# Kudo510/ImageSequenceRegistrationfor6DPoseEstimationLabeling

Measured on AMD Instinct MI355X. Metric: registered images/sec (T-LESS obj 1-like, synthetic) + final Chamfer error, higher is better.
Workload: dtype bf16

## Files before the change

### imagesequenceregistrationfor6dposeestimationlabeling_amd/_capi.py

```python
from __future__ import annotations

import ctypes as C
from pathlib import Path

import torch

import os

_PKG = Path(__file__).resolve().parent
LIB_PATH = Path(os.environ["ISR_HIP_LIB"]) if os.environ.get("ISR_HIP_LIB") else _PKG / "libisr_hip.so"

ISR_OK = 0
ABI_VERSION = 6
DTYPE_BF16 = 0
DTYPE_F32 = 1
DTYPE_BF16_LOG2 = 2
DTYPE_BF16_LOG2_SCREENED = 3
RANSAC_STAGED = 0
RANSAC_SEQUENTIAL = 1
INLIERS_REFIT = 0
INLIERS_RANSAC = 1
FINAL_REFIT = 0
FINAL_EPNP = 1
TUNE = {"nn_path": 0, "nn_filter": 1, "icp_warm": 2, "nn_plan_rq": 3, "nn_plan_blocks": 4,
        "nn_tile_st": 5, "nn_tile_sq": 6, "nn_tile_tb": 7, "ep_wsum_valu": 8, "k1_f32_chain": 9, "k1_split": 10}


class IsrError(RuntimeError):
    pass


_lib = None

_vp = C.c_void_p
_i = C.c_int
_sz = C.c_size_t
_d = C.c_double
_f = C.c_float
_u64 = C.c_uint64
_i64 = C.c_int64

SIGNATURES = {
    "isr_abi_version": (_i, []),
    "isr_last_error": (C.c_char_p, []),
    "isr_device_count": (_i, []),
    "isr_tuning_set": (_i, [_i, _i]),
    "isr_tuning_get": (_i, [_i]),
    "isr_corr_argmax_workspace_bytes": (_sz, [_i, _i, _i, _i]),
    "isr_corr_argmax": (_i, [_vp, _vp, _i, _i, _i, _i, _i, _i, _vp, _vp, _vp, _vp, _sz, _vp]),
    "isr_corr_argmax_digits": (_i, [_vp, _vp, _i, _i, _i, _i, _i, _i, _vp, _vp, _vp, _i, _vp, _vp, _vp, _sz, _vp]),
    "isr_corr_argmax_phase": (_i, [_vp, _vp, _i, _i, _i, _i, _i, _i, _vp, _vp, _vp, _i, _vp, _vp, _i, _vp, _sz, _vp]),
    "isr_corr_argmax_recheck_count": (_i, [_vp, _sz, _i, _i, _i, _vp, _vp]),
    "isr_corr_argmax_recheck_count_f32": (_i, [_vp, _sz, _i, _i, _i, _vp, _vp]),
    "isr_corr_argmax_screen_redone": (_i, [_vp, _sz, _i, _i, _i, _vp, _vp]),
    "isr_corr_quantize_fp6": (_i, [_vp, _i, _i, _vp, _vp, _vp, _vp]),
    "isr_corr_argmax_clock_mhz": (_i, [_vp, _sz, _i, _i, _i, _vp, _vp]),
    "isr_adds_bounds": (_i, [_vp, _i, _vp, _vp, _i, _vp, _vp, _d, _i, _i, _i, _vp, _vp, _vp, _vp]),
    "isr_corr_topk_workspace_bytes": (_sz, [_i, _i]),
    "isr_corr_topk": (_i, [_vp, _vp, _i, _i, _i, _i, _i, _i, _vp, _vp, _vp, _vp, _sz, _vp]),
    "isr_corr_logsoftmax_workspace_bytes": (_sz, [_i, _i, _i, _i]),
    "isr_corr_logsoftmax": (_i, [_vp, _vp, _i, _i, _i, _i, _i, _i, _vp, _i64, _vp, _sz, _vp]),
    "isr_ep_corr_matrices": (_i, [_vp, _vp, _i, _i, _i, _vp, _vp, _vp, _sz, _vp]),
    "isr_mask_bbox": (_i, [_vp, _i, _i, _i, _i, _vp, _vp]),
    "isr_crop_normalize": (_i, [_vp, _vp, _i, _i, _i, _i, _vp, _i, _i, _vp, _vp, _vp, _vp, _vp]),
    "isr_select_top_batch_workspace_bytes": (_sz, [_i, _i]),
    "isr_select_top_batch": (_i, [_vp, _i, _i, _vp, _d, _i, _vp, _vp, _vp, _vp, _sz, _vp]),
# ... 115 lines not shown
```

### imagesequenceregistrationfor6dposeestimationlabeling_amd/csrc/capi_common.hip

```cpp
#include "isr_common.hpp"

#include <atomic>
#include <cstdlib>
#include <cstring>

namespace isr {

char* last_error_buf() {
  static thread_local char buf[512] = {0};
  return buf;
}

void set_error(const char* fmt, ...) {
  va_list ap;
  va_start(ap, fmt);
  vsnprintf(last_error_buf(), 512, fmt, ap);
  va_end(ap);
}

namespace {

struct Tuning {
  std::atomic<int> v[ISR_TUNE_COUNT];
  Tuning() {
    const int defaults[ISR_TUNE_COUNT] = {-1, -1, 1, 0, 0, 0, 0, 0, 0, 0, 0};
    for (int i = 0; i < ISR_TUNE_COUNT; ++i) v[i].store(defaults[i], std::memory_order_relaxed);
    if (const char* e = getenv("ISR_NN_GRID")) { if (e[0] >= '0' && e[0] <= '2') v[ISR_TUNE_NN_PATH] = e[0] - '0'; }
    if (const char* e = getenv("ISR_NN_FILTER")) { if (e[0] == '0' || e[0] == '1') v[ISR_TUNE_NN_FILTER] = e[0] - '0'; }
    if (const char* e = getenv("ISR_ICP_WARM")) { if (e[0] == '0') v[ISR_TUNE_ICP_WARM] = 0; }
    if (const char* e = getenv("ISR_NN_PLAN")) {
      int rq = 0; long want = 0;
      if (sscanf(e, "%d,%ld", &rq, &want) >= 1) {
        if (rq == 1 || rq == 4) v[ISR_TUNE_NN_PLAN_RQ] = rq;
        if (want > 0) v[ISR_TUNE_NN_PLAN_BLOCKS] = (int)want;
      }
    }
    if (const char* e = getenv("ISR_NN_TILE")) {
      double st = 0, sq = 0; int tb = 0;
      (void)sscanf(e, "%lf,%lf,%d", &st, &sq, &tb);
      if (st > 0) v[ISR_TUNE_NN_TILE_ST] = (int)(st * 1000.0 + 0.5);
// ... 97 lines not shown
```

### imagesequenceregistrationfor6dposeestimationlabeling_amd/csrc/corr_argmax.hip

```cpp
#include "isr_common.hpp"

#include <type_traits>

namespace {

using bf16x8 = __attribute__((ext_vector_type(8))) short;
using f16x8 = __attribute__((ext_vector_type(8))) _Float16;
using f32x16 = __attribute__((ext_vector_type(16))) float;

constexpr int kThreads = 256;
constexpr int kWaves = kThreads / 64;
constexpr int kQB = 2;
constexpr int kTK = 128;
constexpr int kChunkStages = 32;
constexpr int kChunk = kTK * kChunkStages;
constexpr float kLog2e = 1.4426950408889634f;
constexpr float kNoM2 = -1.0e30f;
constexpr int kKnBlocks = 64;
constexpr int kRSplitMax = 4;

struct CorrWs {
  float* pm;
  float* pm2;
  int32_t* pbi;
// ... 533 lines not shown
  constexpr int W = 16 * SP;
  const long i = (long)blockIdx.x * 256 + threadIdx.x;
  if (i >= (long)R * W) return;
  const long row = i / W;
  const int d = (int)(i % W);
  const float x = d < D ? X[row * ld + d] * prescale : 0.f;
  if (fabsf(x) > 65000.f) *ovf = 1;
  const _Float16 x1 = (_Float16)x;
  const float r = x - (float)x1;
  const _Float16 x2s = (_Float16)(r * 2048.f);
  const _Float16 x1s = (_Float16)((float)x1 * 4.8828125e-4f);
  uint16_t* o = out + row * (3 * W) + d;
  o[0] = __builtin_bit_cast(uint16_t, x1); o[W] = __builtin_bit_cast(uint16_t, x2s); o[2 * W] = __builtin_bit_cast(uint16_t, x1s);
}

template <bool F16 = false>
__global__ __launch_bounds__(256) void corr_keynorm_kernel(const uint16_t* __restrict__ K, int N, int D,
                                                           int ldk, float inflate, CorrWs ws) {
  __shared__ float red[4];
  if (ws.digits)
    for (int i = blockIdx.x * 256 + threadIdx.x; i < ws.ndigits; i += kKnBlocks * 256) ws.digits[i] = 0;
  if (gated_off(ws)) return;
  float mx = 0.f;
  for (int i = blockIdx.x * 256 + threadIdx.x; i < ws.nhand; i += kKnBlocks * 256) ws.hand[i] = 0;
  for (int n = blockIdx.x * 256 + threadIdx.x; n < N; n += kKnBlocks * 256) {
    const uint16_t* row = K + (size_t)n * ldk;
    float s = 0.f;
    for (int d = 0; d < D; d += 8) {
      const uint4 v = *reinterpret_cast<const uint4*>(row + d);
      const uint32_t w[4] = {v.x, v.y, v.z, v.w};
#pragma unroll
      for (int j = 0; j < 4; ++j) {
        const float lo = elem_f32<F16>((uint16_t)(w[j] & 0xFFFFu)), hi = elem_f32<F16>((uint16_t)(w[j] >> 16));
        s = __builtin_fmaf(lo, lo, s);
        s = __builtin_fmaf(hi, hi, s);
      }
    }
    mx = fmaxf(mx, s);
  }
#pragma unroll
  for (int o = 32; o >= 1; o >>= 1) mx = fmaxf(mx, __shfl_xor(mx, o, 64));
  if ((threadIdx.x & 63) == 0) red[threadIdx.x >> 6] = mx;
  __syncthreads();
  if (threadIdx.x == 0) {
    ws.kn2[blockIdx.x] = fmaxf(fmaxf(red[0], red[1]), fmaxf(red[2], red[3])) * inflate;
    if (blockIdx.x == 0) {
      ws.rcount[0] = 0; ws.rcount[1] = 0; ws.rcount[2] = 0; ws.rcount[3] = 0;
      if (ws.kmax) { ws.kmax[0] = 0u; ws.kmax[1] = 0u; ws.redone[0] = 0ull; ws.redone[1] = 0ull; }
    }
  }
}

__device__ __forceinline__ void digit_count(const CorrWs& ws, int q, float lp) {
  const int img = q / ws.rows_per_image, r = q - img * ws.rows_per_image;
  const bool valid = !ws.n_rows || r < ws.n_rows[img];
  const int key = valid ? img * isr::kDigitBins + (int)(isr::ordered_bits(lp) >> isr::kDigitShift) : -1;
  const int lane = (int)__builtin_amdgcn_mbcnt_hi(~0u, __builtin_amdgcn_mbcnt_lo(~0u, 0u));
  unsigned long long todo = __builtin_amdgcn_ballot_w64(valid);
  while (todo != 0ull) {
    const int leader = (int)__builtin_ctzll(todo);
    const int k = __builtin_amdgcn_readlane(key, leader);
    const unsigned long long same = __builtin_amdgcn_ballot_w64(key == k);
    if (lane == leader) atomicAdd(&ws.digits[k], (int)__builtin_popcountll(same));
    todo &= ~same;
  }
// ... 509 lines not shown
  uint16_t *q2, *k2;
  int32_t* gate;
  CorrWs ws;
  if (route.kind == 1) carve_split(w, P, N, &q2, &k2, &ws);
  else carve_planes(w, P, N, route.sp, route.kind == 3, &q2, &k2, &gate, &ws, nullptr);
  hipStream_t stream = isr::as_stream(stream_);
  int32_t gated = 0;
  if (route.kind == 3) ISR_CHECK_HIP(hipMemcpyAsync(&gated, gate, sizeof(int32_t), hipMemcpyDeviceToHost, stream));
  ISR_CHECK_HIP(hipMemcpyAsync(count_host, ws.rcount, sizeof(int32_t), hipMemcpyDeviceToHost, stream));
  ISR_CHECK_HIP(hipStreamSynchronize(stream));
  if (gated) *count_host = -1;
  return ISR_OK;
}

namespace {

int launch_bf16(const uint16_t* q, const uint16_t* k, int P, int N, int D, int ldq, int ldk, bool log2, const CorrPlan& p,
                const CorrWs& ws, int32_t* idx, float* logp, float* lse, F32Rows f32, float kn_inflate, hipStream_t stream,
                int sp = 0, bool f16 = false, bool screened = false, int phase = 3) {
  const bool ph1 = (phase & 1) != 0, ph2 = (phase & 2) != 0;
  const float eabs = (sp && f16) ? split_eabs(sp) : 0.f;
  const bool lse_only = idx == nullptr;
  const dim3 grid(p.qblocks, p.nsplit);
  const int fin_blocks = (P + 255) / 256;
  const int fin_bf16 = (p.nsplit == 1 && fin_blocks > kFallbackGrid) ? kFallbackGrid : fin_blocks;
  ISR_REQUIRE(sp != 0 || D == 16 || D == 32 || D == 64 || D == 128,
              "isr_corr_argmax(bf16): D=%d must be 16, 32, 64 or 128 (zero-pad the columns)", D);
  ISR_REQUIRE(ldq % 8 == 0 && ldk % 8 == 0 && ((uintptr_t)q % 16 == 0) && ((uintptr_t)k % 16 == 0),
              "isr_corr_argmax(bf16): rows must be 16-byte aligned (ldq=%d ldk=%d)", ldq, ldk);
  ISR_REQUIRE((long long)p.range_chunks * kChunk * ldk * 2 < (1ll << 31),
              "isr_corr_argmax(bf16): a key range of %d rows x ldk=%d exceeds the 2 GiB buffer window",
              p.range_chunks * kChunk, ldk);
  const int cgrid = (int)(((long)p.qblocks * p.nchunks < kFallbackGrid) ? (long)p.qblocks * p.nchunks : kFallbackGrid);
  const dim3 rgrid(16 * kRSplitGrid);
  const double scale = log2 ? 0.6931471805599453094 : 1.0;
  if (ph1) {
    if (f16) corr_keynorm_kernel<true><<<kKnBlocks, 256, 0, stream>>>(k, N, 16 * sp, ldk, kn_inflate, ws);
    else corr_keynorm_kernel<false><<<kKnBlocks, 256, 0, stream>>>(k, N, sp ? 16 * sp : D, ldk, kn_inflate, ws);
  }
#define ISR_LAUNCH_BF16(DKv)                                                                                  \
  do {                                                                                                        \
    if (log2) {                                                                                               \
      if (ph1) {                                                                                              \
      if (lse_only && DKv <= 2)    \
        corr_bf16_direct_kernel<DKv, kQB, false, DKv, 0, false, (DKv <= 2)><<<grid, kThreads, 0, stream>>>(q, k, P, N, ldq, ldk, \
                                                                              p.range_chunks, ws, idx, logp, lse); \
      else                                                                                                    \
      corr_bf16_direct_kernel<DKv, kQB, false><<<grid, kThreads, 0, stream>>>(q, k, P, N, ldq, ldk,          \
                                                                              p.range_chunks, ws, idx, logp, lse); \
      }                                                                                                       \
      if (ph2) {                                                                                              \
      corr_bf16_kernel<DKv, true><<<cgrid, kThreads, 0, stream>>>(q, k, P, N, ldq, ldk, p.range_chunks, p.qblocks,      \
                                                                  p.nchunks, ws);  \
// ... 212 lines not shown
                       false, dg.phase);
  }
  CorrPlan p = make_plan(P, N, slots_for(dtype, D), kWaves * kQB * 32);
  const bool screened = screened_route(dtype, N, D);
  if (screened) {
    p.nsplit = 1;
    p.range_chunks = p.nchunks;
  }
  isr::Workspace w(ws_, ws_bytes);
  CorrWs ws;
  carve(w, P, N, dtype, &ws);
  dg.apply(&ws);
  if (dtype != ISR_DTYPE_F32) {
    return launch_bf16(static_cast<const uint16_t*>(Q), static_cast<const uint16_t*>(K), P, N, D, ldq, ldk,
                       dtype != ISR_DTYPE_BF16, p, ws, idx, logp, lse, F32Rows{nullptr, nullptr, 0, 0, 0}, 1.f, stream, 0, false, screened,
                       dg.phase);
  }
  if (dg.hist && (dg.phase & 1))
    ISR_CHECK_HIP(hipMemsetAsync(dg.hist, 0, sizeof(int32_t) * (size_t)dg.images * isr::kDigitBins, stream));
  return launch_f32_chain(static_cast<const float*>(Q), static_cast<const float*>(K), P, N, D, ldq, ldk, p, ws, idx, logp, lse, stream,
                          dg.phase);
}

}

extern "C" int isr_corr_argmax(const void* Q, const void* K, int P, int N, int D, int ldq, int ldk,
                               int dtype, int32_t* idx, float* logp, float* lse, void* ws_,
                               size_t ws_bytes, isr_stream_t stream_) {
  return corr_argmax_impl(Q, K, P, N, D, ldq, ldk, dtype, idx, logp, lse, ws_, ws_bytes, stream_, DigitArgs{});
}

// ... 34 lines not shown
```

### imagesequenceregistrationfor6dposeestimationlabeling_amd/ops.py

```python
from __future__ import annotations

import ctypes
from dataclasses import dataclass

import numpy as np

import torch

from . import _capi
from ._capi import check, current_stream, lib, ptr, require_cuda

_workspaces: dict[tuple, torch.Tensor] = {}

_timers: dict[str, list] | None = None


def enable_timing(on: bool = True) -> None:
    global _timers
    _timers = {} if on else None


def drain_timing() -> dict[str, tuple[int, float, float]]:
    out = {}
    if _timers is None:
# ... 211 lines not shown
def _pad_cols(t: torch.Tensor, D: int) -> torch.Tensor:
    if t.shape[1] == D:
        return t.contiguous()
    out = torch.zeros((t.shape[0], D), dtype=t.dtype, device=t.device)
    out[:, : t.shape[1]] = t
    return out


LOG2E = 1.4426950408889634


def prescale_queries_log2(queries: torch.Tensor) -> torch.Tensor:
    return (queries.to(torch.float32) * LOG2E).to(torch.bfloat16)


@dataclass
class CorrCall:
    q: torch.Tensor
    k: torch.Tensor
    P: int
    N: int
    Dp: int
    dtype: int
    idx: torch.Tensor
    logp: torch.Tensor
    lse: torch.Tensor | None
    rows_per_image: int
    n_rows: torch.Tensor | None
    hist: torch.Tensor | None
    ws: torch.Tensor
    dev: torch.device

    def outputs(self):
        out = (self.idx, self.logp) if self.lse is None else (self.idx, self.logp, self.lse)
        return out if self.hist is None else out + (self.hist,)


def _corr_prepare(queries, keys, want_lse, log2_prescaled, screened, rows_per_image, n_rows, ws_tag) -> CorrCall:
    dev = require_cuda(queries, keys, n_rows)
    if queries.ndim != 2 or keys.ndim != 2 or queries.shape[1] != keys.shape[1]:
        raise ValueError(f"queries {tuple(queries.shape)} / keys {tuple(keys.shape)} must be (P,D),(N,D)")
    P, D = queries.shape
    N = keys.shape[0]
    if P == 0 or N == 0:
        raise ValueError("empty queries or keys")
    if screened and not log2_prescaled:
        raise ValueError("screened needs log2-prescaled bf16 queries")
    if queries.dtype == torch.bfloat16 and keys.dtype == torch.bfloat16:
        dtype = (_capi.DTYPE_BF16_LOG2_SCREENED if screened else _capi.DTYPE_BF16_LOG2) if log2_prescaled else _capi.DTYPE_BF16
        Dp = next((d for d in (16, 32, 64, 128) if d >= D), None)
        if Dp is None:
            raise ValueError(f"bf16 path supports D <= 128, got {D}")
    else:
        if log2_prescaled:
            raise ValueError("log2_prescaled needs bf16 queries and keys")
        dtype = _capi.DTYPE_F32
        queries, keys = queries.to(torch.float32), keys.to(torch.float32)
        Dp = D
        if D > 128:
            raise ValueError(f"f32 path supports D <= 128, got {D}")
    q, k = _pad_cols(queries, Dp), _pad_cols(keys, Dp)
    idx = torch.empty(P, dtype=torch.int32, device=dev)
    logp = torch.empty(P, dtype=torch.float32, device=dev)
    lse = torch.empty(P, dtype=torch.float32, device=dev) if want_lse else None
    ws = workspace(dev, lib().isr_corr_argmax_workspace_bytes(P, N, Dp, dtype), ws_tag)
    hist = None
    if rows_per_image is not None:
        if rows_per_image <= 0 or P % rows_per_image:
            raise ValueError(f"corr_argmax: P={P} is not a whole number of images of {rows_per_image} rows")
        if n_rows is not None and (n_rows.dtype != torch.int32 or n_rows.numel() != P // rows_per_image):
            raise ValueError("corr_argmax: n_rows must be (images,) int32")
        hist = torch.empty((P // rows_per_image, 2048), dtype=torch.int32, device=dev)
    return CorrCall(q, k, P, N, Dp, dtype, idx, logp, lse, int(rows_per_image or 1), n_rows, hist, ws, dev)


def _corr_launch(c: CorrCall, phase: int, what: str, work: float) -> None:
    L = lib()
    with torch.cuda.device(c.dev), _timed(what, work):
        if phase == 3 and c.hist is None:
            rc = L.isr_corr_argmax(ptr(c.q), ptr(c.k), c.P, c.N, c.Dp, c.Dp, c.Dp, c.dtype, ptr(c.idx), ptr(c.logp), ptr(c.lse),
                                   ptr(c.ws), c.ws.numel(), current_stream(c.dev))
        elif phase == 3:
            rc = L.isr_corr_argmax_digits(ptr(c.q), ptr(c.k), c.P, c.N, c.Dp, c.Dp, c.Dp, c.dtype, ptr(c.idx), ptr(c.logp), ptr(c.lse),
                                          c.rows_per_image, ptr(c.n_rows), ptr(c.hist), ptr(c.ws), c.ws.numel(), current_stream(c.dev))
        else:
            rc = L.isr_corr_argmax_phase(ptr(c.q), ptr(c.k), c.P, c.N, c.Dp, c.Dp, c.Dp, c.dtype, ptr(c.idx), ptr(c.logp), ptr(c.lse),
                                         c.rows_per_image, ptr(c.n_rows), ptr(c.hist), phase, ptr(c.ws), c.ws.numel(),
                                         current_stream(c.dev))
    check(rc, "isr_corr_argmax")
    global _last_corr
    _last_corr = (c.ws, c.P, c.N, c.dtype, c.dev)


def corr_argmax(queries: torch.Tensor, keys: torch.Tensor, want_lse: bool = False,
                log2_prescaled: bool = False, screened: bool = False, rows_per_image: int | None = None,
                n_rows: torch.Tensor | None = None):
    c = _corr_prepare(queries, keys, want_lse, log2_prescaled, screened, rows_per_image, n_rows, "corr")
    _corr_launch(c, 3, "corr_argmax", 2.0 * c.P * c.N * c.Dp)
    return c.outputs()


def corr_argmax_open(queries: torch.Tensor, keys: torch.Tensor, want_lse: bool = False, log2_prescaled: bool = False,
                     screened: bool = False, rows_per_image: int | None = None, n_rows: torch.Tensor | None = None,
                     ws_tag: str = "corr") -> CorrCall:
    c = _corr_prepare(queries, keys, want_lse, log2_prescaled, screened, rows_per_image, n_rows, ws_tag)
    _corr_launch(c, 1, "corr_argmax", 2.0 * c.P * c.N * c.Dp)
    return c


def corr_argmax_close(call: CorrCall):
    _corr_launch(call, 2, "corr_close", 0.0)
    return call.outputs()


def corr_lse(queries: torch.Tensor, keys: torch.Tensor, log2_prescaled: bool = False, screened: bool = False) -> torch.Tensor:
    dev = require_cuda(queries, keys)
    if queries.ndim != 2 or keys.ndim != 2 or queries.shape[1] != keys.shape[1]:
        raise ValueError(f"queries {tuple(queries.shape)} / keys {tuple(keys.shape)} must be (P,D),(N,D)")
    P, D = queries.shape
    N = keys.shape[0]
    if P == 0 or N == 0:
        raise ValueError("empty queries or keys")
    if queries.dtype == torch.bfloat16 and keys.dtype == torch.bfloat16:
        dtype = (_capi.DTYPE_BF16_LOG2_SCREENED if screened else _capi.DTYPE_BF16_LOG2) if log2_prescaled else _capi.DTYPE_BF16
        Dp = next((d for d in (16, 32, 64, 128) if d >= D), None)
        if Dp is None:
            raise ValueError(f"bf16 path supports D <= 128, got {D}")
    else:
        if log2_prescaled:
            raise ValueError("log2_prescaled needs bf16 queries and keys")
        dtype = _capi.DTYPE_F32
        queries, keys = queries.to(torch.float32), keys.to(torch.float32)
        Dp = D
        if D > 128:
            raise ValueError(f"f32 path supports D <= 128, got {D}")
    q, k = _pad_cols(queries, Dp), _pad_cols(keys, Dp)
    lse = torch.empty(P, dtype=torch.float32, device=dev)
    L = lib()
    ws = workspace(dev, L.isr_corr_argmax_workspace_bytes(P, N, Dp, dtype), "corr")
    with torch.cuda.device(dev), _timed("corr_lse", 2.0 * P * N * Dp):
        rc = L.isr_corr_argmax(ptr(q), ptr(k), P, N, Dp, Dp, Dp, dtype, None, None, ptr(lse), ptr(ws), ws.numel(),
                               current_stream(dev))
    check(rc, "isr_corr_argmax (lse only)")
    return lse


def corr_topk(queries: torch.Tensor, keys: torch.Tensor, k: int):
    dev = require_cuda(queries, keys)
    if queries.ndim != 2 or keys.ndim != 2 or queries.shape[1] != keys.shape[1]:
        raise ValueError(f"queries {tuple(queries.shape)} / keys {tuple(keys.shape)} must be (P,D),(N,D)")
    if not 1 <= int(k) <= 8:
# ... 554 lines not shown
```

### imagesequenceregistrationfor6dposeestimationlabeling_amd/sequence.py

```python
from __future__ import annotations

from dataclasses import dataclass

import numpy as np
import torch

from . import ops, pose_est_surf, pose_refine, registration, shard


@dataclass
class SequenceModel:
    keys: torch.Tensor
    pts: torch.Tensor
    log2_queries: bool = False
    screened: bool = False


EPILOGUE_DIGITS = False


@dataclass
class ImageResult:
    pose: torch.Tensor
    status: torch.Tensor
    n_inl: torch.Tensor
    inl_idx: torch.Tensor
    keep: torch.Tensor
    M: torch.Tensor
    idx: torch.Tensor
    logp: torch.Tensor
    n_eval: torch.Tensor | None = None


def register_image(model: SequenceModel, queries: torch.Tensor, pix_xy: torch.Tensor, cam,
                   itr: int = 500, reperr: float = 2.0, seed: int = 0, refine_iters: int = 10,
                   timing: list | None = None, confidence: float = 0.99, loop: str = "staged",
                   inliers: str = "refit", final: str = "refit") -> ImageResult:
    ops._loop_args(loop, inliers, None, final)
    if timing is not None:
        e0, e1 = torch.cuda.Event(enable_timing=True), torch.cuda.Event(enable_timing=True)
        e0.record()
    idx, logp = ops.corr_argmax(queries, model.keys, log2_prescaled=model.log2_queries, screened=model.screened and model.log2_queries)
    if timing is not None:
        e1.record()
        timing.append((e0, e1))
    keep, M, _ = ops.select_top(logp)
    p3d, p2d = ops.gather_corr(idx, keep, M, model.pts, pix_xy)
    r = ops.pnp_ransac(p3d, p2d, cam, H=itr, reperr=reperr, seed=seed, refine_iters=refine_iters, M_dev=M,
                       confidence=confidence, loop=loop, inliers=inliers, final=final)
    return ImageResult(r.pose, r.status, r.n_inl, r.inl_idx, keep, M, idx, logp, r.n_eval)


def register_crop(model: SequenceModel, feat: torch.Tensor, mask: torch.Tensor, cam, c0: int = 0,
                  n_feat: int | None = None, down_sample: int = 3, itr: int = 500, reperr: float = 2.0,
                  seed: int = 0, refine_iters: int = 10, confidence: float = 0.99, loop: str = "staged",
                  inliers: str = "refit", final: str = "refit") -> tuple[ImageResult, torch.Tensor]:
    ops._loop_args(loop, inliers, None, final)
    D = model.keys.shape[1] if n_feat is None else n_feat
    if model.keys.dtype == torch.bfloat16:
        dtype = "bf16_log2" if model.log2_queries else "bf16"
    else:
        dtype = "f32"
    Q, pix, n_dev = ops.prep_queries(feat, mask, c0=c0, D=D, step=down_sample, dtype=dtype)
    keys = model.keys if model.keys.shape[1] == Q.shape[1] else ops._pad_cols(model.keys, Q.shape[1])
    idx, logp = ops.corr_argmax(Q, keys, log2_prescaled=model.log2_queries, screened=model.screened and model.log2_queries)
    keep, M, _ = ops.select_top(logp, n_dev=n_dev)
    p3d, p2d = ops.gather_corr(idx, keep, M, model.pts, pix)
    r = ops.pnp_ransac(p3d, p2d, cam, H=itr, reperr=reperr, seed=seed, refine_iters=refine_iters, M_dev=M,
                       confidence=confidence, loop=loop, inliers=inliers, final=final)
    return ImageResult(r.pose, r.status, r.n_inl, r.inl_idx, keep, M, idx, logp, r.n_eval), n_dev


def register_frame(model: SequenceModel, rgb, mask, camparams, encoder, n_feat: int = 12, down_sample: int = 3,
                   itr: int = 500, reperr: float = 2.0, seed: int = 0, refine_iters: int = 10, confidence: float = 0.99,
                   useMask: bool = True, loop: str = "staged", inliers: str = "refit", final: str = "refit"):
    from . import registration
    ops._loop_args(loop, inliers, None, final)
    inputIM, cropMask, cam, _ = registration.crop_inputs(rgb, mask, camparams, useMask=useMask, down_sample=down_sample)
    with torch.no_grad():
        imfeatsfull = torch.movedim(encoder(inputIM), 1, 3)
# ... 14 lines not shown
    D = model.keys.shape[1] if n_feat is None else n_feat
    if model.keys.dtype == torch.bfloat16:
        dtype = "bf16_log2" if model.log2_queries else "bf16"
    else:
        dtype = "f32"
    cams = np.asarray(cams, np.float64)
    cams = np.broadcast_to(cams, (n, 3, 3)) if cams.ndim == 2 else cams
    seeds = list(range(n)) if seeds is None else list(seeds)
    cur = torch.cuda.current_stream(dev)
    serial = n_streams <= 1
    pool = [cur, cur] if serial else _stream_pool(dev, max(n_streams, 2))
    if not serial:
        for s in pool:
            s.wait_stream(cur)
    k1_stream, side = pool[0], pool[1:]
    out, counts, keys = [], [], None
    for gi, g0 in enumerate(range(0, n, group)):
        g1 = min(n, g0 + group)
        B = g1 - g0
        with torch.cuda.stream(k1_stream):
            Q, pix, n_dev = ops.prep_queries_batch(feats[g0:g1], masks[g0:g1], c0=c0, D=D, step=down_sample, dtype=dtype)
            if keys is None:
                keys = model.keys if model.keys.shape[1] == Q.shape[2] else ops._pad_cols(model.keys, Q.shape[2])
            S = Q.shape[1]
            if EPILOGUE_DIGITS:
                idx_g, logp_g, hist_g = ops.corr_argmax(Q.view(B * S, -1), keys, log2_prescaled=model.log2_queries,
                                                        screened=model.screened and model.log2_queries, rows_per_image=S, n_rows=n_dev)
            else:
                idx_g, logp_g = ops.corr_argmax(Q.view(B * S, -1), keys, log2_prescaled=model.log2_queries,
                                                screened=model.screened and model.log2_queries)
                hist_g = None
            if not serial:
                done = torch.cuda.Event()
                done.record(k1_stream)
        s = side[gi % len(side)]
        if not serial:
            s.wait_event(done)
            for t in (idx_g, logp_g, hist_g, pix, n_dev):
                if t is not None:
                    t.record_stream(s)
        with torch.cuda.stream(s):
            keep, M, _ = ops.select_top_batch(logp_g.view(B, S), n_dev=n_dev, digit_hist=hist_g)
            p3d, p2d = ops.gather_corr_batch(idx_g.view(B, S), keep, M, model.pts, pix)
            r = ops.pnp_ransac_batch(p3d, p2d, cams[g0:g1], M, H=itr, reperr=reperr, seeds=seeds[g0:g1],
                                     refine_iters=refine_iters, confidence=confidence, loop=loop, inliers=inliers, final=final)
# ... 12 lines not shown


def register_frames(model: SequenceModel, rgbs, masks, camparams, encoder, n_feat: int = 12, down_sample: int = 3,
                    itr: int = 500, reperr: float = 2.0, seeds=None, refine_iters: int = 10, confidence: float = 0.99,
                    useMask: bool = True, group: int = 128, loop: str = "staged", inliers: str = "refit", final: str = "refit"):
    ops._loop_args(loop, inliers, None, final)
    inputIM, cropMask, cam, _ = registration.crop_inputs(rgbs, masks, camparams, useMask=useMask, down_sample=down_sample)
    with torch.no_grad():
        imfeatsfull = torch.movedim(encoder(inputIM), 1, 3)
    res, n_dev = register_crops(model, imfeatsfull, cropMask, cam, n_feat=n_feat, down_sample=down_sample, itr=itr,
                                reperr=reperr, seeds=seeds, refine_iters=refine_iters, confidence=confidence, group=group,
                                loop=loop, inliers=inliers, final=final)
    return res, n_dev, cam


def _publish(results: list[ImageResult], consumer: torch.cuda.Stream) -> None:
    for r in results:
        for t in (r.pose, r.status, r.n_inl, r.inl_idx, r.keep, r.M, r.idx, r.logp, r.n_eval):
            if t is not None:
                t.record_stream(consumer)


_streams: dict[tuple, list] = {}
_closed: dict[tuple, torch.cuda.Event] = {}

K1_SPLIT_CLOSE = True


def _stream_pool(dev: torch.device, n: int) -> list:
    key = (dev.index, n)
    if key not in _streams:
        _streams[key] = [torch.cuda.Stream(device=dev, priority=0 if i == 0 else -1) for i in range(n)]
    return _streams[key]


def register_images(model: SequenceModel, images, cam, itr: int = 500, reperr: float = 2.0,
                    seed0: int = 0, refine_iters: int = 10, n_streams: int = 3,
                    confidence: float = 0.99, loop: str = "staged", inliers: str = "refit",
                    final: str = "refit") -> list[ImageResult]:
    ops._loop_args(loop, inliers, None, final)
    dev = model.keys.device
    cur = torch.cuda.current_stream(dev)
    cam_of = (lambda j: cam) if np.ndim(cam) == 2 else (lambda j: cam[j])
    if n_streams <= 1:
        return [register_image(model, q, pix, cam_of(j), itr, reperr, seed0 + j, refine_iters, confidence=confidence,
                               loop=loop, inliers=inliers, final=final)
                for j, (q, pix) in enumerate(images)]
    pool = _stream_pool(dev, n_streams)
    for s in pool:
        s.wait_stream(cur)
    k1_stream, side = pool[0], pool[1:]
    out = []
    for j, (q, pix) in enumerate(images):
        with torch.cuda.stream(k1_stream):
            idx, logp = ops.corr_argmax(q, model.keys, log2_prescaled=model.log2_queries, screened=model.screened and model.log2_queries)
            done = torch.cuda.Event()
            done.record(k1_stream)
        s = side[j % len(side)]
        s.wait_event(done)
        idx.record_stream(s)
        logp.record_stream(s)
        with torch.cuda.stream(s):
            keep, M, _ = ops.select_top(logp)
            p3d, p2d = ops.gather_corr(idx, keep, M, model.pts, pix)
            r = ops.pnp_ransac(p3d, p2d, cam_of(j), H=itr, reperr=reperr, seed=seed0 + j,
                               refine_iters=refine_iters, M_dev=M, confidence=confidence, loop=loop, inliers=inliers, final=final)
        out.append(ImageResult(r.pose, r.status, r.n_inl, r.inl_idx, keep, M, idx, logp, r.n_eval))
    for s in pool:
        cur.wait_stream(s)
    _publish(out, cur)
# ... 14 lines not shown
                        r.n_eval[b:b + 1])
            for b in range(B)]


def register_block(model: SequenceModel, queries: torch.Tensor, pix_xy: torch.Tensor, cam, itr: int = 500,
                   reperr: float = 2.0, seed0: int = 0, refine_iters: int = 10, n_streams: int = 3,
                   group: int = 8, confidence: float = 0.99, loop: str = "staged", inliers: str = "refit",
                   final: str = "refit") -> list[ImageResult]:
    ops._loop_args(loop, inliers, None, final)
    dev = model.keys.device
    n, P = queries.shape[0], queries.shape[1]
    cur = torch.cuda.current_stream(dev)
    cams = np.asarray(cam, np.float64)
    cams = np.broadcast_to(cams, (n, 3, 3)) if cams.ndim == 2 else cams
    pool = _stream_pool(dev, max(n_streams, 2))
    for s in pool:
        s.wait_stream(cur)
    k1_stream, side = pool[0], pool[1:]
    kw = dict(log2_prescaled=model.log2_queries, screened=model.screened and model.log2_queries)
    if EPILOGUE_DIGITS:
        kw["rows_per_image"] = P
    out = []
    for gi, g0 in enumerate(range(0, n, group)):
        g1 = min(n, g0 + group)
        rows = queries[g0:g1].reshape((g1 - g0) * P, -1)
        with torch.cuda.stream(k1_stream):
            if K1_SPLIT_CLOSE:
                tag = f"corr{gi & 1}"
                prev = _closed.get((dev.index, tag))
                if prev is not None:
                    k1_stream.wait_event(prev)
                call = ops.corr_argmax_open(rows, model.keys, ws_tag=tag, **kw)
                res = call.outputs()
            else:
                res = ops.corr_argmax(rows, model.keys, **kw)
            done = torch.cuda.Event()
            done.record(k1_stream)
        s = side[gi % len(side)]
        s.wait_event(done)
        for t in res:
            t.record_stream(s)
        with torch.cuda.stream(s):
            if K1_SPLIT_CLOSE:
# ... 262 lines not shown
```

### include/isr_hip.h

```cpp
#ifndef ISR_HIP_H
#define ISR_HIP_H

#include <stddef.h>
#include <stdint.h>

#ifdef __cplusplus
extern "C" {
#endif

#define ISR_ABI_VERSION 6

#define ISR_OK 0
#define ISR_ERR_ARG (-1)
#define ISR_ERR_WORKSPACE (-2)
#define ISR_ERR_HIP (-3)
#define ISR_ERR_UNSUPPORTED (-4)

#define ISR_DTYPE_BF16 0
#define ISR_DTYPE_F32 1
#define ISR_DTYPE_BF16_LOG2 2

#define ISR_DTYPE_BF16_LOG2_SCREENED 3

typedef void* isr_stream_t;
// ... 1 lines not shown
int isr_abi_version(void);
const char* isr_last_error(void);
int isr_device_count(void);

#define ISR_TUNE_NN_PATH 0
#define ISR_TUNE_NN_FILTER 1
#define ISR_TUNE_ICP_WARM 2
#define ISR_TUNE_NN_PLAN_RQ 3
#define ISR_TUNE_NN_PLAN_BLOCKS 4
#define ISR_TUNE_NN_TILE_ST 5
#define ISR_TUNE_NN_TILE_SQ 6
#define ISR_TUNE_NN_TILE_TB 7
#define ISR_TUNE_EP_WSUM_VALU 8
#define ISR_TUNE_K1_F32_CHAIN 9
#define ISR_TUNE_K1_SPLIT 10
#define ISR_TUNE_COUNT 11
int isr_tuning_set(int knob, int value);
int isr_tuning_get(int knob);

size_t isr_corr_argmax_workspace_bytes(int P, int N, int D, int dtype);
int isr_corr_argmax(const void* Q, const void* K, int P, int N, int D, int ldq, int ldk, int dtype,
                    int32_t* idx, float* logp, float* lse, void* ws, size_t ws_bytes,
                    isr_stream_t stream);

int isr_corr_argmax_digits(const void* Q, const void* K, int P, int N, int D, int ldq, int ldk, int dtype,
                           int32_t* idx, float* logp, float* lse, int rows_per_image, const int32_t* n_rows,
                           int32_t* digit_hist, void* ws, size_t ws_bytes, isr_stream_t stream);

int isr_corr_argmax_phase(const void* Q, const void* K, int P, int N, int D, int ldq, int ldk, int dtype,
                          int32_t* idx, float* logp, float* lse, int rows_per_image, const int32_t* n_rows,
                          int32_t* digit_hist, int phase, void* ws, size_t ws_bytes, isr_stream_t stream);

int isr_corr_argmax_recheck_count(const void* ws, size_t ws_bytes, int P, int N, int dtype,
                                  int32_t* count_host, isr_stream_t stream);
int isr_corr_argmax_recheck_count_f32(const void* ws, size_t ws_bytes, int P, int N, int D, int32_t* count_host,
                                      isr_stream_t stream);

int isr_corr_quantize_fp6(const void* X, int R, int ld, void* out, float* nrm, float* kmax, isr_stream_t stream);

int isr_corr_argmax_screen_redone(const void* ws, size_t ws_bytes, int P, int N, int dtype, long long* count_host,
                                  isr_stream_t stream);

int isr_corr_argmax_clock_mhz(const void* ws, size_t ws_bytes, int P, int N, int dtype, double* mhz_host,
                              isr_stream_t stream);

size_t isr_corr_logsoftmax_workspace_bytes(int P, int N, int D, int dtype);
// ... 173 lines not shown
```

Before: 1104.

## Cache padded keys and per-key norm plan across corr_argmax calls

Result: no change. 1104 (median of 2 runs) (-0.1%).

```diff
diff --git a/imagesequenceregistrationfor6dposeestimationlabeling_amd/_capi.py b/imagesequenceregistrationfor6dposeestimationlabeling_amd/_capi.py
--- a/imagesequenceregistrationfor6dposeestimationlabeling_amd/_capi.py
+++ b/imagesequenceregistrationfor6dposeestimationlabeling_amd/_capi.py
@@ -23,7 +23,7 @@
 FINAL_REFIT = 0
 FINAL_EPNP = 1
 TUNE = {"nn_path": 0, "nn_filter": 1, "icp_warm": 2, "nn_plan_rq": 3, "nn_plan_blocks": 4,
-        "nn_tile_st": 5, "nn_tile_sq": 6, "nn_tile_tb": 7, "ep_wsum_valu": 8, "k1_f32_chain": 9, "k1_split": 10}
+        "nn_tile_st": 5, "nn_tile_sq": 6, "nn_tile_tb": 7, "ep_wsum_valu": 8, "k1_f32_chain": 9, "k1_split": 10, "k1_key_plan": 11}
 
 
 class IsrError(RuntimeError):
@@ -50,6 +50,9 @@
     "isr_corr_argmax": (_i, [_vp, _vp, _i, _i, _i, _i, _i, _i, _vp, _vp, _vp, _vp, _sz, _vp]),
     "isr_corr_argmax_digits": (_i, [_vp, _vp, _i, _i, _i, _i, _i, _i, _vp, _vp, _vp, _i, _vp, _vp, _vp, _sz, _vp]),
     "isr_corr_argmax_phase": (_i, [_vp, _vp, _i, _i, _i, _i, _i, _i, _vp, _vp, _vp, _i, _vp, _vp, _i, _vp, _sz, _vp]),
+    "isr_corr_keys_plan_bytes": (_sz, [_i]),
+    "isr_corr_keys_prepare": (_i, [_vp, _i, _i, _i, _i, _vp, _sz, _vp]),
+    "isr_corr_keys_release": (_i, [_vp]),
     "isr_corr_argmax_recheck_count": (_i, [_vp, _sz, _i, _i, _i, _vp, _vp]),
     "isr_corr_argmax_recheck_count_f32": (_i, [_vp, _sz, _i, _i, _i, _vp, _vp]),
     "isr_corr_argmax_screen_redone": (_i, [_vp, _sz, _i, _i, _i, _vp, _vp]),
diff --git a/imagesequenceregistrationfor6dposeestimationlabeling_amd/csrc/capi_common.hip b/imagesequenceregistrationfor6dposeestimationlabeling_amd/csrc/capi_common.hip
--- a/imagesequenceregistrationfor6dposeestimationlabeling_amd/csrc/capi_common.hip
+++ b/imagesequenceregistrationfor6dposeestimationlabeling_amd/csrc/capi_common.hip
@@ -23,7 +23,7 @@
 struct Tuning {
   std::atomic<int> v[ISR_TUNE_COUNT];
   Tuning() {
-    const int defaults[ISR_TUNE_COUNT] = {-1, -1, 1, 0, 0, 0, 0, 0, 0, 0, 0};
+    const int defaults[ISR_TUNE_COUNT] = {-1, -1, 1, 0, 0, 0, 0, 0, 0, 0, 0, 1};
     for (int i = 0; i < ISR_TUNE_COUNT; ++i) v[i].store(defaults[i], std::memory_order_relaxed);
     if (const char* e = getenv("ISR_NN_GRID")) { if (e[0] >= '0' && e[0] <= '2') v[ISR_TUNE_NN_PATH] = e[0] - '0'; }
     if (const char* e = getenv("ISR_NN_FILTER")) { if (e[0] == '0' || e[0] == '1') v[ISR_TUNE_NN_FILTER] = e[0] - '0'; }
diff --git a/imagesequenceregistrationfor6dposeestimationlabeling_amd/csrc/corr_argmax.hip b/imagesequenceregistrationfor6dposeestimationlabeling_amd/csrc/corr_argmax.hip
--- a/imagesequenceregistrationfor6dposeestimationlabeling_amd/csrc/corr_argmax.hip
+++ b/imagesequenceregistrationfor6dposeestimationlabeling_amd/csrc/corr_argmax.hip
@@ -1,6 +1,8 @@
 #include "isr_common.hpp"
 
+#include <mutex>
 #include <type_traits>
+#include <vector>
 
 namespace {
 
@@ -571,41 +573,74 @@
   o[0] = __builtin_bit_cast(uint16_t, x1); o[W] = __builtin_bit_cast(uint16_t, x2s); o[2 * W] = __builtin_bit_cast(uint16_t, x1s);
 }
 
+template <bool F16>
+__device__ __forceinline__ float key_norm2(const uint16_t* __restrict__ row, int D) {
+  float s = 0.f;
+  for (int d = 0; d < D; d += 8) {
+    const uint4 v = *reinterpret_cast<const uint4*>(row + d);
+    const uint32_t w[4] = {v.x, v.y, v.z, v.w};
+#pragma unroll
+    for (int j = 0; j < 4; ++j) {
+      const float lo = elem_f32<F16>((uint16_t)(w[j] & 0xFFFFu)), hi = elem_f32<F16>((uint16_t)(w[j] >> 16));
+      s = __builtin_fmaf(lo, lo, s);
+      s = __builtin_fmaf(hi, hi, s);
+    }
+  }
+  return s;
+}
+
+__device__ __forceinline__ float block_max256(float mx, float* red) {
+#pragma unroll
+  for (int o = 32; o >= 1; o >>= 1) mx = fmaxf(mx, __shfl_xor(mx, o, 64));
+  if ((threadIdx.x & 63) == 0) red[threadIdx.x >> 6] = mx;
+  __syncthreads();
+  return fmaxf(fmaxf(red[0], red[1]), fmaxf(red[2], red[3]));
+}
+
+constexpr int kPlanHead = kKnBlocks + 16;
+
 template <bool F16 = false>
 __global__ __launch_bounds__(256) void corr_keynorm_kernel(const uint16_t* __restrict__ K, int N, int D,
-                                                           int ldk, float inflate, CorrWs ws) {
+                                                           int ldk, float inflate, const float* __restrict__ plan_kn2, CorrWs ws) {
   __shared__ float red[4];
   if (ws.digits)
     for (int i = blockIdx.x * 256 + threadIdx.x; i < ws.ndigits; i += kKnBlocks * 256) ws.digits[i] = 0;
   if (gated_off(ws)) return;
   float mx = 0.f;
   for (int i = blockIdx.x * 256 + threadIdx.x; i < ws.nhand; i += kKnBlocks * 256) ws.hand[i] = 0;
-  for (int n = blockIdx.x * 256 + threadIdx.x; n < N; n += kKnBlocks * 256) {
-    const uint16_t* row = K + (size_t)n * ldk;
-    float s = 0.f;
-    for (int d = 0; d < D; d += 8) {
-      const uint4 v = *reinterpret_cast<const uint4*>(row + d);
-      const uint32_t w[4] = {v.x, v.y, v.z, v.w};
-#pragma unroll
-      for (int j = 0; j < 4; ++j) {
-        const float lo = elem_f32<F16>((uint16_t)(w[j] & 0xFFFFu)), hi = elem_f32<F16>((uint16_t)(w[j] >> 16));
-        s = __builtin_fmaf(lo, lo, s);
-        s = __builtin_fmaf(hi, hi, s);
-      }
-    }
-    mx = fmaxf(mx, s);
-  }
-#pragma unroll
-  for (int o = 32; o >= 1; o >>= 1) mx = fmaxf(mx, __shfl_xor(mx, o, 64));
-  if ((threadIdx.x & 63) == 0) red[threadIdx.x >> 6] = mx;
-  __syncthreads();
+  if (plan_kn2 == nullptr) {
+    for (int n = blockIdx.x * 256 + threadIdx.x; n < N; n += kKnBlocks * 256) mx = fmaxf(mx, key_norm2<F16>(K + (size_t)n * ldk, D));
+    mx = block_max256(mx, red);
+  } else if (threadIdx.x == 0) {
+    mx = plan_kn2[blockIdx.x];
+  }
   if (threadIdx.x == 0) {
-    ws.kn2[blockIdx.x] = fmaxf(fmaxf(red[0], red[1]), fmaxf(red[2], red[3])) * inflate;
+    ws.kn2[blockIdx.x] = mx * inflate;
     if (blockIdx.x == 0) {
       ws.rcount[0] = 0; ws.rcount[1] = 0; ws.rcount[2] = 0; ws.rcount[3] = 0;
       if (ws.kmax) { ws.kmax[0] = 0u; ws.kmax[1] = 0u; ws.redone[0] = 0ull; ws.redone[1] = 0ull; }
     }
   }
+}
+
+__global__ __launch_bounds__(256) void corr_keys_prepare_kernel(const uint16_t* __restrict__ K, int N, int D, int ldk,
+                                                                float* __restrict__ plan) {
+  __shared__ float red[4];
+  float mx = 0.f;
+  for (int n = blockIdx.x * 256 + threadIdx.x; n < N; n += kKnBlocks * 256) {
+    const float s = key_norm2<false>(K + (size_t)n * ldk, D);
+    plan[kPlanHead + n] = s;
+    mx = fmaxf(mx, s);
+  }
+  mx = block_max256(mx, red);
+  if (threadIdx.x == 0) plan[blockIdx.x] = mx;
+}
+
+__global__ __launch_bounds__(64) void corr_keys_prepare_max_kernel(float* __restrict__ plan) {
+  float v = plan[threadIdx.x];
+#pragma unroll
+  for (int o = 32; o >= 1; o >>= 1) v = fmaxf(v, __shfl_xor(v, o, 64));
+  if (threadIdx.x < kPlanHead - kKnBlocks) plan[kKnBlocks + threadIdx.x] = threadIdx.x == 0 ? v : 0.f;
 }
 
 __device__ __forceinline__ void digit_count(const CorrWs& ws, int q, float lp) {
@@ -1145,10 +1180,63 @@
 }
 
 namespace {
+struct KeyPlanRec { const void* K; int N, D, ldk; const float* plan; };
+std::mutex g_key_plans_mu;
+std::vector<KeyPlanRec> g_key_plans;
+
+const float* key_plan_for(const void* K, int N, int D, int ldk) {
+  if (isr::tuning(ISR_TUNE_K1_KEY_PLAN) == 0) return nullptr;
+  std::lock_guard<std::mutex> lock(g_key_plans_mu);
+  for (const KeyPlanRec& r : g_key_plans)
+    if (r.K == K && r.N == N && r.D == D && r.ldk == ldk) return r.plan;
+  return nullptr;
+}
+}
+
+extern "C" size_t isr_corr_keys_plan_bytes(int N) {
+  return N > 0 ? sizeof(float) * ((size_t)kPlanHead + (size_t)N) : 0;
+}
+
+extern "C" int isr_corr_keys_prepare(const void* K, int N, int D, int ldk, int dtype, isr_corr_keys_plan_t plan, size_t plan_bytes,
+                                     isr_stream_t stream_) {
+  ISR_REQUIRE(K && plan && N > 0, "isr_corr_keys_prepare: null pointer or N=%d", N);
+  ISR_REQUIRE(dtype == ISR_DTYPE_BF16 || dtype == ISR_DTYPE_BF16_LOG2 || dtype == ISR_DTYPE_F32 || dtype == ISR_DTYPE_BF16_LOG2_SCREENED,
+              "isr_corr_keys_prepare: dtype %d", dtype);
+  if (dtype == ISR_DTYPE_F32) {
+    isr::set_error("isr_corr_keys_prepare: f32 keys have no plan (their routes re-derive the plane images and norms per call)");
+    return ISR_ERR_UNSUPPORTED;
+  }
+  ISR_REQUIRE(D == 16 || D == 32 || D == 64 || D == 128, "isr_corr_keys_prepare: D=%d must be 16, 32, 64 or 128 (zero-pad the columns)", D);
+  ISR_REQUIRE(ldk >= D && ldk % 8 == 0 && ((uintptr_t)K % 16 == 0), "isr_corr_keys_prepare: rows must be 16-byte aligned (ldk=%d)", ldk);
+  ISR_REQUIRE((uintptr_t)plan % 16 == 0, "isr_corr_keys_prepare: the plan must be 16-byte aligned");
+  if (plan_bytes < isr_corr_keys_plan_bytes(N)) {
+    isr::set_error("isr_corr_keys_prepare: plan %zu < %zu bytes", plan_bytes, isr_corr_keys_plan_bytes(N));
+    return ISR_ERR_WORKSPACE;
+  }
+  hipStream_t stream = isr::as_stream(stream_);
+  float* pf = static_cast<float*>(plan);
+  corr_keys_prepare_kernel<<<kKnBlocks, 256, 0, stream>>>(static_cast<const uint16_t*>(K), N, D, ldk, pf);
+  corr_keys_prepare_max_kernel<<<1, 64, 0, stream>>>(pf);
+  ISR_CHECK_LAUNCH("key plan kernels");
+  std::lock_guard<std::mutex> lock(g_key_plans_mu);
+  for (KeyPlanRec& r : g_key_plans)
+    if (r.K == K) { r = KeyPlanRec{K, N, D, ldk, pf}; return ISR_OK; }
+  g_key_plans.push_back(KeyPlanRec{K, N, D, ldk, pf});
+  return ISR_OK;
+}
+
+extern "C" int isr_corr_keys_release(const void* K) {
+  std::lock_guard<std::mutex> lock(g_key_plans_mu);
+  for (size_t i = 0; i < g_key_plans.size(); ++i)
+    if (g_key_plans[i].K == K) { g_key_plans.erase(g_key_plans.begin() + (long)i); break; }
+  return ISR_OK;
+}
+
+namespace {
 
 int launch_bf16(const uint16_t* q, const uint16_t* k, int P, int N, int D, int ldq, int ldk, bool log2, const CorrPlan& p,
                 const CorrWs& ws, int32_t* idx, float* logp, float* lse, F32Rows f32, float kn_inflate, hipStream_t stream,
-                int sp = 0, bool f16 = false, bool screened = false, int phase = 3) {
+                int sp = 0, bool f16 = false, bool screened = false, int phase = 3, const float* plan_kn2 = nullptr) {
   const bool ph1 = (phase & 1) != 0, ph2 = (phase & 2) != 0;
   const float eabs = (sp && f16) ? split_eabs(sp) : 0.f;
   const bool lse_only = idx == nullptr;
@@ -1166,8 +1254,8 @@
   const dim3 rgrid(16 * kRSplitGrid);
   const double scale = log2 ? 0.6931471805599453094 : 1.0;
   if (ph1) {
-    if (f16) corr_keynorm_kernel<true><<<kKnBlocks, 256, 0, stream>>>(k, N, 16 * sp, ldk, kn_inflate, ws);
-    else corr_keynorm_kernel<false><<<kKnBlocks, 256, 0, stream>>>(k, N, sp ? 16 * sp : D, ldk, kn_inflate, ws);
+    if (f16) corr_keynorm_kernel<true><<<kKnBlocks, 256, 0, stream>>>(k, N, 16 * sp, ldk, kn_inflate, plan_kn2, ws);
+    else corr_keynorm_kernel<false><<<kKnBlocks, 256, 0, stream>>>(k, N, sp ? 16 * sp : D, ldk, kn_inflate, plan_kn2, ws);
   }
 #define ISR_LAUNCH_BF16(DKv)                                                                                  \
   do {                                                                                                        \
@@ -1410,7 +1498,7 @@
   if (dtype != ISR_DTYPE_F32) {
     return launch_bf16(static_cast<const uint16_t*>(Q), static_cast<const uint16_t*>(K), P, N, D, ldq, ldk,
                        dtype != ISR_DTYPE_BF16, p, ws, idx, logp, lse, F32Rows{nullptr, nullptr, 0, 0, 0}, 1.f, stream, 0, false, screened,
-                       dg.phase);
+                       dg.phase, (dg.phase & 1) ? key_plan_for(K, N, D, ldk) : nullptr);
   }
   if (dg.hist && (dg.phase & 1))
     ISR_CHECK_HIP(hipMemsetAsync(dg.hist, 0, sizeof(int32_t) * (size_t)dg.images * isr::kDigitBins, stream));
diff --git a/imagesequenceregistrationfor6dposeestimationlabeling_amd/ops.py b/imagesequenceregistrationfor6dposeestimationlabeling_amd/ops.py
--- a/imagesequenceregistrationfor6dposeestimationlabeling_amd/ops.py
+++ b/imagesequenceregistrationfor6dposeestimationlabeling_amd/ops.py
@@ -1,6 +1,7 @@
 from __future__ import annotations
 
 import ctypes
+import weakref
 from dataclasses import dataclass
 
 import numpy as np
@@ -249,6 +250,76 @@
     return (queries.to(torch.float32) * LOG2E).to(torch.bfloat16)
 
 
+def _keys_sig(t: torch.Tensor) -> tuple:
+    return (t.device.index, t.data_ptr(), tuple(t.shape), tuple(t.stride()), t.dtype, t._version)
+
+
+_live_plans: dict[int, "weakref.ref[KeyPlan]"] = {}
+
+
+class KeyPlan:
+
+    def __init__(self, keys: torch.Tensor):
+        dev = require_cuda(keys)
+        if keys.ndim != 2 or keys.shape[0] == 0:
+            raise ValueError(f"keys {tuple(keys.shape)} must be (N,D), N > 0")
+        self.sig = _keys_sig(keys)
+        self.keys = keys
+        self.k = self.buf = self.ready = None
+        if keys.dtype != torch.bfloat16:
+            return
+        Dp = next((d for d in (16, 32, 64, 128) if d >= keys.shape[1]), None)
+        if Dp is None:
+            raise ValueError(f"bf16 path supports D <= 128, got {keys.shape[1]}")
+        self.k = _pad_cols(keys, Dp)
+        self.k_version = self.k._version
+        N, L = keys.shape[0], lib()
+        old = _live_plans.get(self.k.data_ptr())
+        if old is not None and old() is not None:
+            old().release()
+        self.buf = torch.empty(L.isr_corr_keys_plan_bytes(N), dtype=torch.uint8, device=dev)
+        with torch.cuda.device(dev):
+            rc = L.isr_corr_keys_prepare(ptr(self.k), N, Dp, Dp, _capi.DTYPE_BF16, ptr(self.buf), self.buf.numel(), current_stream(dev))
+            check(rc, "isr_corr_keys_prepare")
+            self.ready = torch.cuda.Event()
+            self.ready.record()
+        self._key = self.k.data_ptr()
+        _live_plans[self._key] = weakref.ref(self)
+
+    def matches(self, keys: torch.Tensor) -> bool:
+        if self.k is not None and self.k._version != self.k_version:
+            return False
+        return keys is self.k or _keys_sig(keys) == self.sig
+
+    def norms(self) -> torch.Tensor:
+        return self.buf.view(torch.float32)[80:80 + self.keys.shape[0]]
+
+    def max_norm(self) -> torch.Tensor:
+        return self.buf.view(torch.float32)[64]
+
+    def release(self) -> None:
+        key = self.__dict__.pop("_key", None)
+        if key is not None:
+            ref = _live_plans.get(key)
+            if ref is not None and ref() not in (self, None):
+                return
+            _live_plans.pop(key, None)
+            lib().isr_corr_keys_release(key)
+
+    def __del__(self):
+        try:
+            self.release()
+        except Exception:
+            pass
+
+
+def _drop_stale_plan(k: torch.Tensor, using: KeyPlan | None) -> None:
+    ref = _live_plans.get(k.data_ptr())
+    pl = ref() if ref is not None else None
+    if pl is not None and pl is not using and (pl.k._version != pl.k_version or tuple(pl.k.shape) != tuple(k.shape)):
+        pl.release()
+
+
 @dataclass
 class CorrCall:
     q: torch.Tensor
@@ -265,14 +336,20 @@
     hist: torch.Tensor | None
     ws: torch.Tensor
     dev: torch.device
+    plan: KeyPlan | None = None
 
     def outputs(self):
         out = (self.idx, self.logp) if self.lse is None else (self.idx, self.logp, self.lse)
         return out if self.hist is None else out + (self.hist,)
 
 
-def _corr_prepare(queries, keys, want_lse, log2_prescaled, screened, rows_per_image, n_rows, ws_tag) -> CorrCall:
+def _corr_prepare(queries, keys, want_lse, log2_prescaled, screened, rows_per_image, n_rows, ws_tag, key_plan=None) -> CorrCall:
     dev = require_cuda(queries, keys, n_rows)
+    if key_plan is not None:
+        if not key_plan.matches(keys):
+            raise ValueError("corr_argmax: the key plan is stale (the keys were written, moved or reshaped since it was made)")
+        if key_plan.k is not None:
+            torch.cuda.current_stream(dev).wait_event(key_plan.ready)
     if queries.ndim != 2 or keys.ndim != 2 or queries.shape[1] != keys.shape[1]:
         raise ValueError(f"queries {tuple(queries.shape)} / keys {tuple(keys.shape)} must be (P,D),(N,D)")
     P, D = queries.shape
@@ -294,7 +371,12 @@
         Dp = D
         if D > 128:
             raise ValueError(f"f32 path supports D <= 128, got {D}")
-    q, k = _pad_cols(queries, Dp), _pad_cols(keys, Dp)
+    q = _pad_cols(queries, Dp)
+    if key_plan is not None and key_plan.k is not None and dtype != _capi.DTYPE_F32:
+        k = key_plan.k
+    else:
+        k = _pad_cols(keys, Dp)
+    _drop_stale_plan(k, key_plan)
     idx = torch.empty(P, dtype=torch.int32, device=dev)
     logp = torch.empty(P, dtype=torch.float32, device=dev)
     lse = torch.empty(P, dtype=torch.float32, device=dev) if want_lse else None
@@ -306,7 +388,7 @@
         if n_rows is not None and (n_rows.dtype != torch.int32 or n_rows.numel() != P // rows_per_image):
             raise ValueError("corr_argmax: n_rows must be (images,) int32")
         hist = torch.empty((P // rows_per_image, 2048), dtype=torch.int32, device=dev)
-    return CorrCall(q, k, P, N, Dp, dtype, idx, logp, lse, int(rows_per_image or 1), n_rows, hist, ws, dev)
+    return CorrCall(q, k, P, N, Dp, dtype, idx, logp, lse, int(rows_per_image or 1), n_rows, hist, ws, dev, key_plan)
 
 
 def _corr_launch(c: CorrCall, phase: int, what: str, work: float) -> None:
@@ -329,21 +411,25 @@
 
 def corr_argmax(queries: torch.Tensor, keys: torch.Tensor, want_lse: bool = False,
                 log2_prescaled: bool = False, screened: bool = False, rows_per_image: int | None = None,
-                n_rows: torch.Tensor | None = None):
-    c = _corr_prepare(queries, keys, want_lse, log2_prescaled, screened, rows_per_image, n_rows, "corr")
+                n_rows: torch.Tensor | None = None, key_plan: KeyPlan | None = None):
+    c = _corr_prepare(queries, keys, want_lse, log2_prescaled, screened, rows_per_image, n_rows, "corr", key_plan)
     _corr_launch(c, 3, "corr_argmax", 2.0 * c.P * c.N * c.Dp)
     return c.outputs()
 
 
 def corr_argmax_open(queries: torch.Tensor, keys: torch.Tensor, want_lse: bool = False, log2_prescaled: bool = False,
                      screened: bool = False, rows_per_image: int | None = None, n_rows: torch.Tensor | None = None,
-                     ws_tag: str = "corr") -> CorrCall:
-    c = _corr_prepare(queries, keys, want_lse, log2_prescaled, screened, rows_per_image, n_rows, ws_tag)
+                     ws_tag: str = "corr", key_plan: KeyPlan | None = None) -> CorrCall:
+    c = _corr_prepare(queries, keys, want_lse, log2_prescaled, screened, rows_per_image, n_rows, ws_tag, key_plan)
     _corr_launch(c, 1, "corr_argmax", 2.0 * c.P * c.N * c.Dp)
     return c
 
 
 def corr_argmax_close(call: CorrCall):
+    s = torch.cuda.current_stream(call.dev)
+    for t in (call.ws, call.q, call.k, call.n_rows):
+        if t is not None:
+            t.record_stream(s)
     _corr_launch(call, 2, "corr_close", 0.0)
     return call.outputs()
 
@@ -370,6 +456,7 @@
         if D > 128:
             raise ValueError(f"f32 path supports D <= 128, got {D}")
     q, k = _pad_cols(queries, Dp), _pad_cols(keys, Dp)
+    _drop_stale_plan(k, None)
     lse = torch.empty(P, dtype=torch.float32, device=dev)
     L = lib()
     ws = workspace(dev, L.isr_corr_argmax_workspace_bytes(P, N, Dp, dtype), "corr")
diff --git a/imagesequenceregistrationfor6dposeestimationlabeling_amd/sequence.py b/imagesequenceregistrationfor6dposeestimationlabeling_amd/sequence.py
--- a/imagesequenceregistrationfor6dposeestimationlabeling_amd/sequence.py
+++ b/imagesequenceregistrationfor6dposeestimationlabeling_amd/sequence.py
@@ -14,6 +14,13 @@
     pts: torch.Tensor
     log2_queries: bool = False
     screened: bool = False
+
+    def key_plan(self) -> ops.KeyPlan:
+        pl = self.__dict__.get("_key_plan")
+        if pl is None or not pl.matches(self.keys):
+            pl = ops.KeyPlan(self.keys)
+            self.__dict__["_key_plan"] = pl
+        return pl
 
 
 EPILOGUE_DIGITS = False
@@ -40,7 +47,8 @@
     if timing is not None:
         e0, e1 = torch.cuda.Event(enable_timing=True), torch.cuda.Event(enable_timing=True)
         e0.record()
-    idx, logp = ops.corr_argmax(queries, model.keys, log2_prescaled=model.log2_queries, screened=model.screened and model.log2_queries)
+    idx, logp = ops.corr_argmax(queries, model.keys, log2_prescaled=model.log2_queries, screened=model.screened and model.log2_queries,
+                                key_plan=model.key_plan())
     if timing is not None:
         e1.record()
         timing.append((e0, e1))
@@ -62,8 +70,8 @@
     else:
         dtype = "f32"
     Q, pix, n_dev = ops.prep_queries(feat, mask, c0=c0, D=D, step=down_sample, dtype=dtype)
-    keys = model.keys if model.keys.shape[1] == Q.shape[1] else ops._pad_cols(model.keys, Q.shape[1])
-    idx, logp = ops.corr_argmax(Q, keys, log2_prescaled=model.log2_queries, screened=model.screened and model.log2_queries)
+    keys, plan = _planned_keys(model, Q.shape[1])
+    idx, logp = ops.corr_argmax(Q, keys, log2_prescaled=model.log2_queries, screened=model.screened and model.log2_queries, key_plan=plan)
     keep, M, _ = ops.select_top(logp, n_dev=n_dev)
     p3d, p2d = ops.gather_corr(idx, keep, M, model.pts, pix)
     r = ops.pnp_ransac(p3d, p2d, cam, H=itr, reperr=reperr, seed=seed, refine_iters=refine_iters, M_dev=M,
@@ -108,21 +116,22 @@
         for s in pool:
             s.wait_stream(cur)
     k1_stream, side = pool[0], pool[1:]
-    out, counts, keys = [], [], None
+    out, counts, keys, plan = [], [], None, None
     for gi, g0 in enumerate(range(0, n, group)):
         g1 = min(n, g0 + group)
         B = g1 - g0
         with torch.cuda.stream(k1_stream):
             Q, pix, n_dev = ops.prep_queries_batch(feats[g0:g1], masks[g0:g1], c0=c0, D=D, step=down_sample, dtype=dtype)
             if keys is None:
-                keys = model.keys if model.keys.shape[1] == Q.shape[2] else ops._pad_cols(model.keys, Q.shape[2])
+                keys, plan = _planned_keys(model, Q.shape[2])
             S = Q.shape[1]
             if EPILOGUE_DIGITS:
                 idx_g, logp_g, hist_g = ops.corr_argmax(Q.view(B * S, -1), keys, log2_prescaled=model.log2_queries,
-                                                        screened=model.screened and model.log2_queries, rows_per_image=S, n_rows=n_dev)
+                                                        screened=model.screened and model.log2_queries, rows_per_image=S, n_rows=n_dev,
+                                                        key_plan=plan)
             else:
                 idx_g, logp_g = ops.corr_argmax(Q.view(B * S, -1), keys, log2_prescaled=model.log2_queries,
-                                                screened=model.screened and model.log2_queries)
+                                                screened=model.screened and model.log2_queries, key_plan=plan)
                 hist_g = None
             if not serial:
                 done = torch.cuda.Event()
@@ -165,6 +174,15 @@
     return res, n_dev, cam
 
 
+def _planned_keys(model: SequenceModel, width: int):
+    plan = model.key_plan()
+    if plan.k is not None and plan.k.shape[1] == width:
+        return plan.k, plan
+    if model.keys.shape[1] == width:
+        return model.keys, plan
+    return ops._pad_cols(model.keys, width), None
+
+
 def _publish(results: list[ImageResult], consumer: torch.cuda.Stream) -> None:
     for r in results:
         for t in (r.pose, r.status, r.n_inl, r.inl_idx, r.keep, r.M, r.idx, r.logp, r.n_eval):
@@ -174,6 +192,7 @@
 
 _streams: dict[tuple, list] = {}
 _closed: dict[tuple, torch.cuda.Event] = {}
+_opened: dict[int, int] = {}
 
 K1_SPLIT_CLOSE = True
 
@@ -198,13 +217,15 @@
                                loop=loop, inliers=inliers, final=final)
                 for j, (q, pix) in enumerate(images)]
     pool = _stream_pool(dev, n_streams)
+    plan = model.key_plan()
     for s in pool:
         s.wait_stream(cur)
     k1_stream, side = pool[0], pool[1:]
     out = []
     for j, (q, pix) in enumerate(images):
         with torch.cuda.stream(k1_stream):
-            idx, logp = ops.corr_argmax(q, model.keys, log2_prescaled=model.log2_queries, screened=model.screened and model.log2_queries)
+            idx, logp = ops.corr_argmax(q, model.keys, log2_prescaled=model.log2_queries, screened=model.screened and model.log2_queries,
+                                        key_plan=plan)
             done = torch.cuda.Event()
             done.record(k1_stream)
         s = side[j % len(side)]
@@ -249,10 +270,11 @@
     cams = np.asarray(cam, np.float64)
     cams = np.broadcast_to(cams, (n, 3, 3)) if cams.ndim == 2 else cams
     pool = _stream_pool(dev, max(n_streams, 2))
+    plan = model.key_plan()
     for s in pool:
         s.wait_stream(cur)
     k1_stream, side = pool[0], pool[1:]
-    kw = dict(log2_prescaled=model.log2_queries, screened=model.screened and model.log2_queries)
+    kw = dict(log2_prescaled=model.log2_queries, screened=model.screened and model.log2_queries, key_plan=plan)
     if EPILOGUE_DIGITS:
         kw["rows_per_image"] = P
     out = []
@@ -261,7 +283,9 @@
         rows = queries[g0:g1].reshape((g1 - g0) * P, -1)
         with torch.cuda.stream(k1_stream):
             if K1_SPLIT_CLOSE:
-                tag = f"corr{gi & 1}"
+                count = _opened.get(dev.index, 0)
+                _opened[dev.index] = count + 1
+                tag = f"corr{count & 1}"
                 prev = _closed.get((dev.index, tag))
                 if prev is not None:
                     k1_stream.wait_event(prev)
diff --git a/include/isr_hip.h b/include/isr_hip.h
--- a/include/isr_hip.h
+++ b/include/isr_hip.h
@@ -39,7 +39,8 @@
 #define ISR_TUNE_EP_WSUM_VALU 8
 #define ISR_TUNE_K1_F32_CHAIN 9
 #define ISR_TUNE_K1_SPLIT 10
-#define ISR_TUNE_COUNT 11
+#define ISR_TUNE_K1_KEY_PLAN 11
+#define ISR_TUNE_COUNT 12
 int isr_tuning_set(int knob, int value);
 int isr_tuning_get(int knob);
 
@@ -55,6 +56,12 @@
 int isr_corr_argmax_phase(const void* Q, const void* K, int P, int N, int D, int ldq, int ldk, int dtype,
                           int32_t* idx, float* logp, float* lse, int rows_per_image, const int32_t* n_rows,
                           int32_t* digit_hist, int phase, void* ws, size_t ws_bytes, isr_stream_t stream);
+
+typedef void* isr_corr_keys_plan_t;
+size_t isr_corr_keys_plan_bytes(int N);
+int isr_corr_keys_prepare(const void* K, int N, int D, int ldk, int dtype, isr_corr_keys_plan_t plan, size_t plan_bytes,
+                          isr_stream_t stream);
+int isr_corr_keys_release(const void* K);
 
 int isr_corr_argmax_recheck_count(const void* ws, size_t ws_bytes, int P, int N, int dtype,
                                   int32_t* count_host, isr_stream_t stream);
```
